# ForJadeForest/DistillCLIP

Hardware: AMD Instinct MI355X
Metric: image-text pairs/sec (distill step) (higher is better)
Workload: dtype bf16; 1 GPU; l_clip.yaml dual distill: ViT-B/32 CLIP teacher -> weight-shared ViT(6x768,24h,R2) + text(4x768,12h,R2) students, 224px/77tok, losses out_l1+out_cos+0.1*cos_diff, fwd+loss+bwd+AdamW; global_batch=512, batch_per_gpu=512, parallelism=dp1, gradient_exchange=none, negatives=local (reference training_step semantics), optimizer_in_step=True, teacher_residual=fp16, saved_gelu_derivative=u8 fixed point, clock_probe=True

## Files before the change

distillclip_amd/csrc/gemm_common.h:

```cpp
#pragma once
#include <math.h>
#include <stdlib.h>
#include "common.h"
#include <type_traits>

namespace dgemm {

constexpr int BM = 128, BN = 128, BK = 64;
constexpr int SUB = 1024;
constexpr int HT = 16384;

inline unsigned long long* g_gemm_stamps = nullptr;

struct GemmNT {
    const bf16_t* A; int64_t lda;
    const bf16_t* B; int64_t ldb;
    void* C; int64_t ldc;
    int M, N, K;
    float alpha;
    const float* bias;
    const void* aux_in;
    void* aux_out;
    const void* residual; int64_t ldr;
    int row_group; const float* rowadd;
// ... 76 lines not shown
        float dg[8];
#pragma unroll
        for (int e = 0; e < 8; ++e) {
            const float sg = __builtin_amdgcn_rcpf(1.f + __expf(-1.702f * v[e]));
            dg[e] = fmaf(1.702f * v[e] * sg, 1.f - sg, sg);
            v[e] *= sg;
        }
        if (LEAN || p.aux_out) *(uint2*)((uint8_t*)p.aux_out + o) = uint2{dg_pack4(dg[0], dg[1], dg[2], dg[3]), dg_pack4(dg[4], dg[5], dg[6], dg[7])};
    }
    if (MODE == 3 || (!LEAN && p.residual)) {
        if (OUT == 2) {
            const f16x8 r = sd.rh;
#pragma unroll
            for (int e = 0; e < 8; ++e) v[e] += (float)r[e];
        } else {
            float4 r0, r1;
            if (OUT == 1) { r0 = sd.r0; r1 = sd.r1; }
            else {
                const float* rp = (const float*)p.residual + orr;
                r0 = *(const float4*)rp; r1 = *(const float4*)(rp + 4);
            }
            v[0] += r0.x; v[1] += r0.y; v[2] += r0.z; v[3] += r0.w; v[4] += r1.x; v[5] += r1.y; v[6] += r1.z; v[7] += r1.w;
        }
    }
    if (OUT == 1) {
        float* cp = (float*)p.C + o;
        *(float4*)cp = float4{v[0], v[1], v[2], v[3]};
        *(float4*)(cp + 4) = float4{v[4], v[5], v[6], v[7]};
    } else if (OUT == 2) {
        f16x8 ov;
#pragma unroll
        for (int e = 0; e < 8; ++e) ov[e] = (_Float16)v[e];
        *(f16x8*)((_Float16*)p.C + o) = ov;
    } else {
        bf16x8 ov;
#pragma unroll
        for (int e = 0; e < 8; ++e) ov[e] = f2bf(v[e]);
        *(bf16x8*)((bf16_t*)p.C + o) = ov;
    }
    if (CSUM_ALWAYS || (OUT == 0 && (MODE == 2 || (MODE == 0 && p.colsum)))) {
#pragma unroll
        for (int e = 0; e < 8; ++e) csum[e] += v[e];
    }
}

#define WAIT_VMCNT(n) asm volatile("s_waitcnt vmcnt(" #n ")" ::: "memory")
#define WAIT_LGKM0() asm volatile("s_waitcnt lgkmcnt(0)" ::: "memory")

__device__ __forceinline__ void wg_stamp(unsigned long long* const& stamps, const int& tid, int k) {
    if (stamps && tid == 0) {
        if (k == 3) WAIT_VMCNT(0);
        stamps[6 * (int64_t)blockIdx.x + k] = __builtin_readcyclecounter();
        if (k == 0) stamps[6 * (int64_t)blockIdx.x + 4] = __builtin_amdgcn_s_memrealtime();
        if (k == 3) stamps[6 * (int64_t)blockIdx.x + 5] = __builtin_amdgcn_s_memrealtime();
    }
}

__device__ __forceinline__ void mfma_4x4(f32x4 (&acc)[4][4], const bf16x8 (&a)[4], const bf16x8 (&b)[4]) {
#pragma unroll
    for (int i = 0; i < 4; ++i)
#pragma unroll
        for (int j = 0; j < 4; ++j) acc[i][j] = __builtin_amdgcn_mfma_f32_16x16x32_bf16(a[i], b[j], acc[i][j], 0, 0, 0);
}

template <bool SWAP>
__device__ __forceinline__ f32x4 mfma_rc(bf16x8 rowf, bf16x8 colf, f32x4 c) {
    return SWAP ? __builtin_amdgcn_mfma_f32_16x16x32_bf16(colf, rowf, c, 0, 0, 0) : __builtin_amdgcn_mfma_f32_16x16x32_bf16(rowf, colf, c, 0, 0, 0);
}
#define PHASE_MFMA(SWAP, acc, R0, RT, af, b0, b1)                                                                         \
    do {                                                                                                                  \
        __builtin_amdgcn_s_barrier();                                                                                     \
        __builtin_amdgcn_s_setprio(1);                                                                                    \
        _Pragma("unroll") for (int kb_ = 0; kb_ < 2; ++kb_)                                                               \
            _Pragma("unroll") for (int i_ = 0; i_ < (RT); ++i_) {                                                         \
                _Pragma("unroll") for (int j_ = 0; j_ < 2; ++j_)                                                          \
                    acc[(R0) + i_][j_] = mfma_rc<SWAP>(af[i_][kb_], b0[j_][kb_], acc[(R0) + i_][j_]);                     \
                _Pragma("unroll") for (int j_ = 0; j_ < 2; ++j_)                                                          \
                    acc[(R0) + i_][2 + j_] = mfma_rc<SWAP>(af[i_][kb_], b1[j_][kb_], acc[(R0) + i_][2 + j_]);             \
            }                                                                                                             \
        __builtin_amdgcn_s_setprio(0);                                                                                    \
        __builtin_amdgcn_s_barrier();                                                                                     \
    } while (0)

template <int NI, int LD>
__device__ __forceinline__ void stage_acc(float* cs, const f32x4 (*acc)[4], int row0, int col0, int lane) {
#pragma unroll
    for (int i = 0; i < NI; ++i)
#pragma unroll
        for (int j = 0; j < 4; ++j)
#pragma unroll
            for (int r = 0; r < 4; ++r) cs[(row0 + i * 16 + (lane >> 4) * 4 + r) * LD + col0 + j * 16 + (lane & 15)] = acc[i][j][r];
}

}
```

distillclip_amd/csrc/gemm_nt.hip:

```cpp

#include "gemm_common.h"
#include <atomic>

using namespace dgemm;

namespace {

constexpr int TILE_BYTES = (BM / 16) * (BK / 32) * SUB;
constexpr int CLD = BN + 4;
constexpr int NT_LDS = (4 * TILE_BYTES > BM * CLD * 4) ? 4 * TILE_BYTES : BM * CLD * 4;


__device__ __forceinline__ void stage_operand(const bf16_t* __restrict__ G, int64_t ld, int row0, int rows_max,
                                              int k0, char* lds_tile, int wave, int lane) {
    const int L = lane * 16;
    const int X = swz(L);
    const int r = X >> 6, c = (X >> 4) & 3;
#pragma unroll
    for (int s = 0; s < 4; ++s) {
        const int sub = wave * 4 + s;
        const int rb = sub >> 1, kb = sub & 1;
        int row = row0 + rb * 16 + r;
        row = row < rows_max ? row : rows_max - 1;
        const bf16_t* src = G + (int64_t)row * ld + (k0 + kb * 32 + c * 8);
        __builtin_amdgcn_global_load_lds((gbl_void*)src, (lds_void*)(lds_tile + sub * SUB), 16, 0, 0);
    }
}

template <int ACT, int OUT>
__global__ __launch_bounds__(256) void gemm_nt_kernel(GemmNT p) {
    extern __shared__ __attribute__((aligned(16))) char smem[];
    const int tid = threadIdx.x, lane = tid & 63;
    const int wave = __builtin_amdgcn_readfirstlane(tid >> 6);
    const int wm = wave >> 1, wn = wave & 1;

    const int nwg = p.tiles_m * p.tiles_n;
    const int t = xcd_remap(blockIdx.x, nwg);
    const int tm = t / p.tiles_n, tn = t % p.tiles_n;
    const int m0 = tm * BM, n0 = tn * BN;

    char* As = smem;
    char* Bs = smem + 2 * TILE_BYTES;

    f32x4 acc[4][4];
#pragma unroll
    for (int i = 0; i < 4; ++i)
#pragma unroll
        for (int j = 0; j < 4; ++j) acc[i][j] = f32x4{0.f, 0.f, 0.f, 0.f};

    const int nk = p.K / BK;
    stage_operand(p.A, p.lda, m0, p.M, 0, As, wave, lane);
    stage_operand(p.B, p.ldb, n0, p.N, 0, Bs, wave, lane);

    const int fragoff = swz((lane & 15) * 64 + (lane >> 4) * 16);

    for (int kt = 0; kt < nk; ++kt) {
        __syncthreads();
        if (kt + 1 < nk) {
            const int nb = (kt + 1) & 1;
            stage_operand(p.A, p.lda, m0, p.M, (kt + 1) * BK, As + nb * TILE_BYTES, wave, lane);
            stage_operand(p.B, p.ldb, n0, p.N, (kt + 1) * BK, Bs + nb * TILE_BYTES, wave, lane);
        }
        const char* a_t = As + (kt & 1) * TILE_BYTES;
        const char* b_t = Bs + (kt & 1) * TILE_BYTES;
#pragma unroll
        for (int kb = 0; kb < 2; ++kb) {
            bf16x8 af[4], bfr[4];
#pragma unroll
            for (int i = 0; i < 4; ++i)
                af[i] = *(const bf16x8*)(a_t + ((wm * 4 + i) * 2 + kb) * SUB + fragoff);
#pragma unroll
            for (int j = 0; j < 4; ++j)
                bfr[j] = *(const bf16x8*)(b_t + ((wn * 4 + j) * 2 + kb) * SUB + fragoff);
            mfma_4x4(acc, af, bfr);
        }
    }

    __syncthreads();
    float* cs = (float*)smem;
    stage_acc<4, CLD>(cs, acc, wm * 64, wn * 64, lane);
    __syncthreads();
    const int cc = (tid & 15) * 8;
    const int col = n0 + cc;
    const bool col_ok = col < p.N;
    float bias[8], csum[8];
#pragma unroll
    for (int e = 0; e < 8; ++e) { bias[e] = 0.f; csum[e] = 0.f; }
    if (p.bias && col_ok) {
        const float4 b0 = *(const float4*)(p.bias + col), b1 = *(const float4*)(p.bias + col + 4);
        bias[0] = b0.x; bias[1] = b0.y; bias[2] = b0.z; bias[3] = b0.w; bias[4] = b1.x; bias[5] = b1.y; bias[6] = b1.z; bias[7] = b1.w;
    }
#pragma unroll
    for (int it = 0; it < 8; ++it) {
        const int rl = (tid >> 4) + it * 16;
        const int row = m0 + rl;
        if (row >= p.M || !col_ok) break;
        const float4 c0 = *(const float4*)(cs + rl * CLD + cc), c1 = *(const float4*)(cs + rl * CLD + cc + 4);
        float v[8] = {c0.x, c0.y, c0.z, c0.w, c1.x, c1.y, c1.z, c1.w};
        const int64_t o = (int64_t)row * p.ldc + col, orr = (int64_t)row * p.ldr + col;
        EpiSide sd;
        epilogue_load_side<ACT, OUT>(p, o, orr, sd);
        epilogue_vec8<ACT, OUT, 0, true>(p, v, row, col, o, orr, bias, csum, sd);
    }
    if (p.colsum) {
        __syncthreads();
#pragma unroll
        for (int e = 0; e < 8; ++e) cs[(tid >> 4) * CLD + cc + e] = csum[e];
        __syncthreads();
        if (tid < BN && n0 + tid < p.N) {
            float x = 0.f;
#pragma unroll
            for (int r = 0; r < 16; ++r) x += cs[r * CLD + tid];
            unsafeAtomicAdd(p.colsum + n0 + tid, x);
        }
    }
}


constexpr int nt256_lds(int mi) { return 2 * (2 * HT + 2 * (mi * 16 * BK * 2)); }

__device__ __forceinline__ void stage_half_perm(const bf16_t* __restrict__ G, int64_t ld, int row0, int rows_max, int k0,
                                                char* buf, int wave, int lane) {
    const int L = lane * 16;
    const int X = swz(L);
    const int r = X >> 6, c = (X >> 4) & 3;
    const int j = wave & 3;
    int row = row0 + (wave >> 2) * 64 + (j >> 1) * 32 + (r >> 2) * 8 + (j & 1) * 4 + (r & 3);
    row = row < rows_max ? row : rows_max - 1;
    const bf16_t* src = G + (int64_t)row * ld + k0 + c * 8;
    __builtin_amdgcn_global_load_lds((gbl_void*)src, (lds_void*)(buf + (wave * 2 + 0) * SUB), 16, 0, 0);
    __builtin_amdgcn_global_load_lds((gbl_void*)(src + 32), (lds_void*)(buf + (wave * 2 + 1) * SUB), 16, 0, 0);
}

template <int RH>
__device__ __forceinline__ void stage_rowhalf(const bf16_t* __restrict__ G, int64_t ld, int m0, int rows_max, int k0,
                                              char* abase, int hta, int dn, int wave, int lane) {
    const int L = lane * 16;
    const int X = swz(L);
    const int r = X >> 6, c = (X >> 4) & 3;
    constexpr int AROWS = RH * 32;
    {
        const int wv = RH == 3 ? wave % 6 : wave;
        const int g = wv / RH, i = wv % RH + dn * RH;
        int row = m0 + g * AROWS + i * 16 + r;
        row = row < rows_max ? row : rows_max - 1;
        const bf16_t* src = G + (int64_t)row * ld + k0 + c * 8;
        char* dst = abase + g * hta + (i * 2) * SUB;
        __builtin_amdgcn_global_load_lds((gbl_void*)src, (lds_void*)dst, 16, 0, 0);
        __builtin_amdgcn_global_load_lds((gbl_void*)(src + 32), (lds_void*)(dst + SUB), 16, 0, 0);
    }
    if (RH == 5) {
        const int e = wave & 3, rbk = 8 + (e >> 1), kb = e & 1;
        const int g = rbk / RH, i = rbk % RH + dn * RH;
        int row = m0 + g * AROWS + i * 16 + r;
        row = row < rows_max ? row : rows_max - 1;
        const bf16_t* src = G + (int64_t)row * ld + k0 + kb * 32 + c * 8;
        __builtin_amdgcn_global_load_lds((gbl_void*)src, (lds_void*)(abase + g * hta + (i * 2 + kb) * SUB), 16, 0, 0);
    }
}

__device__ __forceinline__ float row16_sum(float x) {
    auto dpp = [](float v, auto ctrl) {
        return __builtin_bit_cast(float, __builtin_amdgcn_update_dpp(0, __builtin_bit_cast(int, v), decltype(ctrl)::value, 0xf, 0xf, false));
    };
    x += dpp(x, std::integral_constant<int, 0xB1>{});
    x += dpp(x, std::integral_constant<int, 0x4E>{});
    x += dpp(x, std::integral_constant<int, 0x141>{});
    x += dpp(x, std::integral_constant<int, 0x140>{});
    return x;
}

template <int ACT, int OUT, int MI>
__global__ __launch_bounds__(512) void gemm_nt256_kernel(GemmNT p) {
    extern __shared__ __attribute__((aligned(16))) char smem[];
    constexpr int RH = MI / 2;
    constexpr int AROWS = MI * 16;
    constexpr int HTA = AROWS * BK * 2;
    constexpr int PAR = nt256_lds(MI) / 2;
    constexpr int BMT = 2 * AROWS;
    const int tid = threadIdx.x, lane = tid & 63;
    const int wave = __builtin_amdgcn_readfirstlane(tid >> 6);
    const int wr = wave >> 2, wc = wave & 3;

    const int nwg = p.tiles_m * p.tiles_n;
    const int nk = p.K / BK;
    const int nload = 4 * nk;
    int m0, n0;
    auto locate = [&](int tl) {
        const int t = xcd_remap(tl, nwg);
        int tm, tn;
        if (p.group_n >= p.tiles_n) { tm = t / p.tiles_n; tn = t % p.tiles_n; }
        else {
            const int per = p.tiles_m * p.group_n;
            const int gi = t / per, rem = t - gi * per;
            const int left = p.tiles_n - gi * p.group_n;
            const int gw = left < p.group_n ? left : p.group_n;
            tm = rem / gw; tn = gi * p.group_n + rem % gw;
        }
// ... 61 lines not shown
    if (wr == 0) __builtin_amdgcn_s_barrier();
    wg_stamp(p.stamps, tid, 2);
    const int g = lane >> 4, rl = lane & 15;

    const int colb = n0 + wc * 64 + g * 8;
    float bias[2][8], csum[2][8];
#pragma unroll
    for (int jp = 0; jp < 2; ++jp) {
#pragma unroll
        for (int e = 0; e < 8; ++e) { bias[jp][e] = 0.f; csum[jp][e] = 0.f; }
        const int col = colb + jp * 32;
        if (p.bias && col < p.N) {
            const float4 q0 = *(const float4*)(p.bias + col), q1 = *(const float4*)(p.bias + col + 4);
            bias[jp][0] = q0.x; bias[jp][1] = q0.y; bias[jp][2] = q0.z; bias[jp][3] = q0.w;
            bias[jp][4] = q1.x; bias[jp][5] = q1.y; bias[jp][6] = q1.z; bias[jp][7] = q1.w;
        }
    }
    constexpr bool OUT_F32 = OUT == 1;
    constexpr bool SIDE = OUT != 0 || ACT == 3 || ACT == 4;
    constexpr int NU = 2 * MI;
    constexpr int BU = !SIDE ? NU : (OUT_F32 ? ((ACT == 3 || ACT == 4) ? 4 : (MI == 8 ? 8 : (MI == 6 ? 6 : 5))) : (MI == 10 ? 10 : NU));
    static_assert(NU % BU == 0, "batch size must divide the unit count");
    EpiSide side[SIDE ? BU : 1];
    const int row0 = m0 + wr * AROWS + rl;
    const int64_t o0 = (int64_t)row0 * p.ldc + colb, r0off = (int64_t)row0 * p.ldr + colb;
    const int64_t ostep = 16 * p.ldc, rstep = 16 * p.ldr;
    const bool full = m0 + BMT <= p.M && n0 + 256 <= p.N;
    auto run_units = [&](auto mode_tag) {
        constexpr int MODE = decltype(mode_tag)::value;
#pragma unroll
        for (int ub = 0; ub < NU; ub += BU) {
            if (SIDE) {
#pragma unroll
                for (int u = ub; u < ub + BU; ++u) {
                    const int i = u >> 1, jp = u & 1;
                    if (full || (row0 + i * 16 < p.M && colb + jp * 32 < p.N))
                        epilogue_load_side<ACT, OUT>(p, o0 + i * ostep + jp * 32, r0off + i * rstep + jp * 32, side[u - ub]);
                }
            }
#pragma unroll
            for (int u = ub; u < ub + BU; ++u) {
                const int i = u >> 1, jp = u & 1;
                const int row = row0 + i * 16, col = colb + jp * 32;
                if (full || (row < p.M && col < p.N)) {
                    float v[8];
#pragma unroll
                    for (int r = 0; r < 4; ++r) { v[r] = acc[i][2 * jp][r]; v[4 + r] = acc[i][2 * jp + 1][r]; }
                    epilogue_vec8<ACT, OUT, MODE>(p, v, row, col, o0 + i * ostep + jp * 32, r0off + i * rstep + jp * 32, bias[jp], csum[jp],
                                                      side[SIDE ? u - ub : 0]);
                }
            }
        }
    };
    const bool lean = p.row_group == 0 && ((ACT == 5 || ACT == 6) ? p.aux_out != nullptr : p.aux_out == nullptr) && (OUT != 0 ? p.residual != nullptr : p.residual == nullptr);
    if constexpr (OUT != 0) {
        if (lean) run_units(std::integral_constant<int, 3>{});
        else run_units(std::integral_constant<int, 0>{});
    } else if constexpr (ACT == 3 || ACT == 4) {
        if (lean && p.colsum) run_units(std::integral_constant<int, 2>{});
        else run_units(std::integral_constant<int, 0>{});
    } else {
        if (lean && !p.colsum) run_units(std::integral_constant<int, 1>{});
        else if (lean) run_units(std::integral_constant<int, 2>{});
        else run_units(std::integral_constant<int, 0>{});
    }
    if (OUT == 0 && p.colsum) {
        float* cs = (float*)smem;
#pragma unroll
        for (int jp = 0; jp < 2; ++jp)
#pragma unroll
            for (int e = 0; e < 8; ++e) {
                const float x = row16_sum(csum[jp][e]);
                if (rl == 0) cs[wr * 256 + wc * 64 + jp * 32 + g * 8 + e] = x;
            }
        WAIT_LGKM0();
        __builtin_amdgcn_s_barrier();
        const int tc = wave * 64 + lane;
        if (tc < 256 && n0 + tc < p.N) unsafeAtomicAdd(p.colsum + n0 + tc, cs[tc] + cs[256 + tc]);
    }
    wg_stamp(p.stamps, tid, 3);
    if (p.clk && blockIdx.x == 0 && tid == 0) { p.clk[2] = __builtin_amdgcn_s_memtime(); p.clk[3] = __builtin_amdgcn_s_memrealtime(); }
}

bool use_256(const GemmNT& p) {
    static const int mode = [] { const char* e = getenv("DCLIP_GEMM256"); return e ? atoi(e) : 1; }();
    return mode != 0 && p.M >= 1024 && p.N >= 256;
}

std::atomic<unsigned long long*> g_clock_buf{nullptr};
std::atomic<long long> g_clock_cap{0};
std::atomic<long long> g_clock_count{0};
inline unsigned long long* next_clock_slot() {
    unsigned long long* buf = g_clock_buf.load(std::memory_order_acquire);
    const long long cap = g_clock_cap.load(std::memory_order_relaxed);
    if (!buf || cap <= 0) return nullptr;
    return buf + 4 * (g_clock_count.fetch_add(1, std::memory_order_relaxed) % cap);
}

int tile_height_mi(const GemmNT& p, int act, int out) {
    static const int mode320 = [] { const char* e = getenv("DCLIP_GEMM320"); return e ? atoi(e) : 1; }();
    if (!mode320) return 8;
    if (mode320 == 2) return 10;
    if (mode320 == 6) return 6;
    const int tn = (p.N + 255) / 256;
    const double nkt = (double)(p.K / BK), e8 = out == 1 ? 40000.0 : out == 2 ? 24000.0 : (act == 0 || act == 4 ? 9500.0 : 14000.0);
    auto cost = [&](int rows, double per_kt, double escale) {
        const int tmx = (p.M + rows - 1) / rows;
        return (double)((tmx * tn + 255) / 256) * (3300.0 + nkt * per_kt + escale * e8);
    };
    const double c8 = cost(256, 2750.0, 1.0), c10 = cost(320, 3200.0, 1.25), c6 = cost(192, 2150.0, 0.75);
    int mi = 8;
    if (c10 < c8) mi = 10;
    if (c6 < (mi == 10 ? c10 : c8) * 0.97) mi = 6;
    return mi;
}

int raster_group_n(const GemmNT& p) {
    const int tn = p.tiles_n, ntiles = p.tiles_m * p.tiles_n;
    const double panel = 512.0 * (double)p.K, a_bytes = 2.0 * (double)p.M * (double)p.K;
    double best = 0.0; int best_g = tn;
    for (int g = 1; g <= tn; ++g) {
        const int ngroups = (tn + g - 1) / g;
        const double b_term = (g * panel <= 2.5e6) ? 8.0 * g * panel * (ngroups > 8 ? ngroups / 8.0 : 1.0)
                                                   : (double)ntiles / 32.0 * g * panel;
        const double cost = a_bytes * ngroups + b_term;
        if (g == 1 || cost < best * 0.999) { best = cost; best_g = g; }
    }
    return best_g;
}

template <int ACT, int MI>
void launch_nt256(const GemmNT& p, int out, hipStream_t st) {
    const dim3 grid(p.tiles_m * p.tiles_n), block(512);
    constexpr size_t lds = nt256_lds(MI) + 16;
    if (out == 1) { if constexpr (ACT == 0) hipLaunchKernelGGL((gemm_nt256_kernel<0, 1, MI>), grid, block, lds, st, p); }
    else if (out == 2) { if constexpr (ACT == 0) hipLaunchKernelGGL((gemm_nt256_kernel<0, 2, MI>), grid, block, lds, st, p); }
    else hipLaunchKernelGGL((gemm_nt256_kernel<ACT, 0, MI>), grid, block, lds, st, p);
}

template <int ACT>
int launch_nt(GemmNT p, int out, hipStream_t st) {
    if constexpr (ACT != 0) { if (out == 2) { dclip_set_error("dclip_gemm_nt: f16 output needs act = DCLIP_ACT_NONE"); return DCLIP_EINVAL; } }
    if (use_256(p) && !(out != 0 && p.colsum) && (ACT == 0 || out == 0)) {
        const int mi = tile_height_mi(p, ACT, out);
        p.tiles_m = (p.M + mi * 32 - 1) / (mi * 32); p.tiles_n = (p.N + 255) / 256;
        p.clk = next_clock_slot();
        p.group_n = raster_group_n(p);
        if (mi == 10) launch_nt256<ACT, 10>(p, out, st);
        else if (mi == 6) launch_nt256<ACT, 6>(p, out, st);
        else launch_nt256<ACT, 8>(p, out, st);
        return dclip_check_launch("dclip_gemm_nt");
    }
    const int grid = p.tiles_m * p.tiles_n;
    const size_t lds = NT_LDS;
    if (out == 1) hipLaunchKernelGGL((gemm_nt_kernel<ACT, 1>), dim3(grid), dim3(256), lds, st, p);
    else if (out == 2) { if constexpr (ACT == 0) hipLaunchKernelGGL((gemm_nt_kernel<0, 2>), dim3(grid), dim3(256), lds, st, p); }
    else hipLaunchKernelGGL((gemm_nt_kernel<ACT, 0>), dim3(grid), dim3(256), lds, st, p);
    return dclip_check_launch("dclip_gemm_nt");
}

}

extern "C" int dclip_trace_gemm_stamps(void* buf) { g_gemm_stamps = (unsigned long long*)buf; return 0; }
extern "C" int64_t dclip_trace_gemm_clock(void* buf, int64_t cap) {
    const long long n = g_clock_count.exchange(0, std::memory_order_relaxed);
    g_clock_cap.store(buf ? (long long)cap : 0, std::memory_order_relaxed);
    g_clock_buf.store((unsigned long long*)buf, std::memory_order_release);
    return (int64_t)n;
}

extern "C" int dclip_gemm_nt(const void* A, int64_t lda, const void* B, int64_t ldb, void* C, int64_t ldc,
                             int64_t M, int64_t N, int64_t K, float alpha, const float* bias, int act,
                             const void* aux_in, void* aux_out, const void* residual, int64_t ldr, int out_dtype,
                             int64_t row_group, const float* rowadd, float* colsum_acc, void* stream) {
    DCLIP_REQUIRE(A && B && C, "dclip_gemm_nt: null operand");
    DCLIP_REQUIRE(M > 0 && N > 0 && K > 0, "dclip_gemm_nt: empty problem M=%ld N=%ld K=%ld", (long)M, (long)N, (long)K);
    DCLIP_REQUIRE(K % BK == 0, "dclip_gemm_nt: K=%ld must be a multiple of %d", (long)K, BK);
    DCLIP_REQUIRE(lda % 8 == 0 && ldb % 8 == 0 && ((uintptr_t)A % 16) == 0 && ((uintptr_t)B % 16) == 0,
                  "dclip_gemm_nt: operand rows must be 16-byte aligned (lda=%ld ldb=%ld)", (long)lda, (long)ldb);
    DCLIP_REQUIRE(N % 8 == 0 && ldc % 8 == 0 && ((uintptr_t)C % 16) == 0, "dclip_gemm_nt: N and ldc must be multiples of 8 and C 16-byte aligned (N=%ld ldc=%ld)", (long)N, (long)ldc);
    DCLIP_REQUIRE(out_dtype >= 0 && out_dtype <= 2, "dclip_gemm_nt: bad output dtype %d (0 bf16, 1 f32, 2 f16)", out_dtype);
    DCLIP_REQUIRE(!residual || (ldr % (out_dtype == 2 ? 8 : 4) == 0 && ((uintptr_t)residual % 16) == 0), "dclip_gemm_nt: residual rows must be 16-byte aligned");
    DCLIP_REQUIRE(act >= 0 && act <= 6, "dclip_gemm_nt: bad activation code %d", act);
    DCLIP_REQUIRE(out_dtype != 2 || act == 0, "dclip_gemm_nt: f16 output needs act = DCLIP_ACT_NONE");
    DCLIP_REQUIRE((act != DCLIP_ACT_DGELU && act != DCLIP_ACT_MULAUX) || aux_in, "dclip_gemm_nt: DGELU / MULAUX need aux_in");
    DCLIP_REQUIRE(!aux_in || ((uintptr_t)aux_in % 16) == 0, "dclip_gemm_nt: aux_in must be 16-byte aligned");
    DCLIP_REQUIRE(!aux_out || ((uintptr_t)aux_out % 16) == 0, "dclip_gemm_nt: aux_out must be 16-byte aligned");
    DCLIP_REQUIRE(row_group == 0 || rowadd, "dclip_gemm_nt: row_group needs rowadd");
    DCLIP_REQUIRE(M < (1LL << 31) && N < (1LL << 31), "dclip_gemm_nt: dimension overflow");
    GemmNT p;
    p.A = (const bf16_t*)A; p.lda = lda; p.B = (const bf16_t*)B; p.ldb = ldb; p.C = C; p.ldc = ldc;
    p.M = (int)M; p.N = (int)N; p.K = (int)K; p.alpha = alpha; p.bias = bias;
    p.aux_in = aux_in; p.aux_out = aux_out; p.residual = residual; p.ldr = ldr;
    p.row_group = (int)row_group; p.rowadd = rowadd; p.colsum = colsum_acc;
    p.tiles_m = (int)((M + BM - 1) / BM); p.tiles_n = (int)((N + BN - 1) / BN);
    p.stamps = g_gemm_stamps;
    p.group_n = 1 << 30;
    p.clk = nullptr;
    hipStream_t st = (hipStream_t)stream;
    const int out_f32 = out_dtype == 1;
    const double aux_b = (act == DCLIP_ACT_MULAUX || act == DCLIP_ACT_GELU_SAVE || act == DCLIP_ACT_QUICKGELU_SAVE) ? 1.0 : 2.0;
    TraceScope tr(DCLIP_TRACE_GEMM_NT, 2.0 * (double)M * (double)N * (double)K,
                  2.0 * ((double)M * K + (double)N * K) + ((out_f32 ? 4.0 : 2.0) + (residual ? (out_dtype == 2 ? 2.0 : 4.0) : 0.0) + (aux_in ? aux_b : 0.0) + (aux_out ? aux_b : 0.0)) * (double)M * N,
                  stream, (int)M, (int)N, (int)K,
                  act + 8 * (out_f32 != 0) + 16 * (residual != nullptr) + 32 * (colsum_acc != nullptr) + 64 * (out_dtype == 2));
    switch (act) {
        case 0: return launch_nt<0>(p, out_dtype, st);
        case 1: return launch_nt<1>(p, out_dtype, st);
        case 2: return launch_nt<2>(p, out_dtype, st);
        case 3: return launch_nt<3>(p, out_dtype, st);
        case 4: return launch_nt<4>(p, out_dtype, st);
        case 5: return launch_nt<5>(p, out_dtype, st);
        default: return launch_nt<6>(p, out_dtype, st);
    }
}
```

include/dclip.h:

```cpp
#ifndef DCLIP_H
#define DCLIP_H
#include <stddef.h>
#include <stdint.h>
#ifdef __cplusplus
extern "C" {
#endif

#define DCLIP_OK 0
#define DCLIP_EINVAL (-1)
#define DCLIP_ELAUNCH (-2)

int dclip_version(void);
int dclip_runtime_check(void);
const char* dclip_arch(void);
const char* dclip_last_error_string(void);

#define DCLIP_ACT_NONE 0
#define DCLIP_ACT_QUICKGELU 1
#define DCLIP_ACT_GELU 2
#define DCLIP_ACT_DGELU 3
#define DCLIP_ACT_MULAUX 4
#define DCLIP_ACT_GELU_SAVE 5
#define DCLIP_ACT_QUICKGELU_SAVE 6
#define DCLIP_OUT_BF16 0
#define DCLIP_OUT_F32 1
#define DCLIP_OUT_F16 2

int dclip_gemm_nt(const void* A, int64_t lda, const void* B, int64_t ldb, void* C, int64_t ldc,
                  int64_t M, int64_t N, int64_t K, float alpha, const float* bias, int act,
                  const void* aux_in, void* aux_out, const void* residual, int64_t ldr, int out_dtype,
                  int64_t row_group, const float* rowadd, float* colsum_acc, void* stream);

size_t dclip_gemm_tn_workspace_bytes(void);
int64_t dclip_gemm_tn_atomic_fallbacks(void);
int dclip_gemm_tn_acc(const void* A, int64_t lda, const void* B, int64_t ldb, float* dW, int64_t ldo,
                      int64_t M, int64_t P, int64_t Q, int splits, void* workspace, size_t ws_bytes, void* stream);

int dclip_colsum_acc(const void* X, int64_t ld, float* db, int64_t M, int64_t N, void* stream);

int dclip_layernorm_fwd(const float* x, int64_t ldx, const int32_t* row_index, const float* gamma, const float* beta,
                        void* y, int64_t ldy, int out_f32, float* mean, float* rstd, int64_t M, int64_t D, float eps,
                        void* stream);
int dclip_layernorm_fwd_f16(const void* x, int64_t ldx, const int32_t* row_index, const float* gamma, const float* beta,
                            void* y, int64_t ldy, int out_dtype, float* mean, float* rstd, int64_t M, int64_t D, float eps,
                            void* stream);
int dclip_layernorm_bwd(const void* dy, int64_t lddy, int dy_f32, const float* x, int64_t ldx, const int32_t* row_index,
                        const float* gamma, const float* mean, const float* rstd, float* dx_acc, int64_t lddx,
                        void* dx_bf16, int64_t lddb, float* dgamma, float* dbeta, float* colsum_acc, int64_t M, int64_t D,
                        void* stream);

int dclip_attn_nt(const void* A, int64_t lda, const void* Bm, int64_t ldb, void* C, int out_f32, int64_t B, int64_t H,
                  int64_t N, int64_t Np, int64_t hd, float alpha, void* stream);
int dclip_attn_nn(const void* A, const void* Bm, int64_t ldb, void* C, int64_t ldc, int64_t B, int64_t H, int64_t N,
                  int64_t Np, int64_t hd, float alpha, int a_blocked, void* stream);
int dclip_attn_tn(const void* A, const void* Bm, int64_t ldb, void* C, int64_t ldc, int64_t B, int64_t H, int64_t N,
                  int64_t Np, int64_t hd, float alpha, int a_blocked, void* stream);
int dclip_attn_fused_fwd(const void* qkv, int64_t ldq, void* ctx, int64_t ldc, int64_t B, int64_t H, int64_t N, int64_t hd,
                         float scale, int causal, void* stream);
int dclip_attn_stream_fwd(const void* qkv, int64_t ldq, void* ctx, int64_t ldc, int64_t B, int64_t H, int64_t N, int64_t hd,
                          float scale, void* stream);
int dclip_attn_softmax_fwd(const float* S, const float* Wl, const float* Ww, void* P, void* R, int64_t B, int64_t H,
                           int64_t N, int64_t Np, int causal, void* stream);
int dclip_attn_softmax_bwd(const void* dR, const void* P, const void* S, int scores_bf16, const float* Wl, const float* Ww,
                           void* dS, float* dWl, float* dWw, int64_t B, int64_t H, int64_t N, int64_t Np, void* stream);
int dclip_attn_mix_supported(int64_t H, int64_t N, int64_t hd);
size_t dclip_attn_mix_bwd_workspace_bytes(int64_t B, int64_t H, int64_t N);
void dclip_attn_mix_debug_stamps(void* fwd, void* bwd_a, void* bwd_b);
int dclip_attn_mix_fwd(const void* qkv, int64_t ld, const float* Wl, const float* Ww, void* R, float* stats, int64_t B, int64_t H,
                       int64_t N, int64_t Np, int64_t hd, float scale, void* stream);
int dclip_attn_mix_bwd(const void* qkv, int64_t ld, const void* dO, int64_t ldo, const float* Wl, const float* Ww,
                       const float* stats, void* dS, float* dWl, float* dWw, void* workspace, size_t ws_bytes, int64_t B, int64_t H,
                       int64_t N, int64_t Np, int64_t hd, float scale, void* stream);
int dclip_attn_nn_rows(const void* A, const void* Bm, int64_t ldb, void* C, int64_t ldc, int64_t B, int64_t H, int64_t N, int64_t Np,
                       int64_t hd, float alpha, int a_blocked, const int32_t* pick, int fill_zero, void* stream);
int dclip_attn_tn_rows(const void* A, const void* Bm, int64_t ldb, void* C, int64_t ldc, int64_t B, int64_t H, int64_t N, int64_t Np,
                       int64_t hd, float alpha, int a_blocked, const int32_t* pick, void* stream);
int dclip_attn_fused_fwd_rows(const void* qkv, int64_t ldq, void* ctx, int64_t ldc, int64_t B, int64_t H, int64_t N, int64_t hd,
                              float scale, int causal, const int32_t* pick, void* stream);
int dclip_attn_mix_fwd_rows(const void* qkv, int64_t ld, const float* Wl, const float* Ww, void* R, float* stats, int64_t B, int64_t H,
                            int64_t N, int64_t Np, int64_t hd, float scale, const int32_t* pick, void* stream);
int dclip_attn_mix_bwd_rows(const void* qkv, int64_t ld, const void* dO, int64_t ldo, const float* Wl, const float* Ww,
                            const float* stats, void* dS, float* dWl, float* dWw, void* workspace, size_t ws_bytes, int64_t B, int64_t H,
                            int64_t N, int64_t Np, int64_t hd, float scale, const int32_t* pick, void* stream);
int dclip_attn_maps_fwd(const void* qkv, int64_t ld, const float* Wl, float* score_map, float* prob_map, int64_t B, int64_t H, int64_t N,
                        int64_t hd, float scale, int causal, void* stream);
size_t dclip_attn_maps_bwd_workspace_bytes(int64_t B, int64_t H, int64_t N);
int dclip_attn_maps_bwd(const void* qkv, int64_t ld, const float* Wl, const float* d_score_map, const float* d_prob_map, void* dS,
                        int ds_blocked, float* dWl, void* workspace, size_t ws_bytes, int64_t B, int64_t H, int64_t N, int64_t Np,
                        int64_t hd, float scale, int causal, void* stream);

int dclip_cast_bf16(const float* src, void* dst, int64_t n, void* stream);
int dclip_cast_f16_f32(const void* src, float* dst, int64_t n, void* stream);
int dclip_axpy_f32(float* dst, const float* src, void* dst_bf16, int64_t n, float* colsum_acc, int64_t D, void* stream);
int dclip_cast_transpose_bf16_multi(const float* const* W, void* const* Wb, void* const* Wt, const int64_t* R, const int64_t* C,
                                    int64_t n, void* stream);
int dclip_im2row(const float* img, void* rows, int64_t B, int64_t C, int64_t res, int64_t patch, int cls_rows, void* stream);
int dclip_im2row_ld(const float* img, void* rows, int64_t ldk, int64_t B, int64_t C, int64_t res, int64_t patch, int cls_rows,
                    void* stream);
int dclip_token_table(const float* pos, const float* cls, const float* bias, float* out, int64_t ntok, int64_t D, void* stream);
int dclip_token_table_bwd(const float* tok_sum, float* dpos, float* dcls, float* dbias, int64_t ntok, int64_t D, int has_cls,
                          void* stream);
int dclip_batch_sum_acc(const float* G, float* out, int64_t B, int64_t N, int64_t D, void* stream);
int dclip_embed_gather(const int64_t* ids, int64_t id_stride, const float* table, const float* pos, void* out, int out_dtype,
                       int64_t rows, int64_t N, int64_t D, void* stream);
int dclip_embed_scatter_add(const int64_t* ids, const void* dx, int dx_f32, float* dtable, int64_t rows, int64_t D,
                            int64_t vocab, void* stream);
int dclip_pick_index(const int64_t* ids, int64_t id_stride, int32_t* idx, int64_t B, int64_t N, void* stream);
int dclip_adamw(float* p, float* g, float* m, float* v, int64_t n, float lr, float beta1, float beta2, float eps,
                float weight_decay, int64_t step, int zero_grad, void* stream);
#define DCLIP_ADAMW_MAX_RANGES 24
int dclip_adamw_multi(float* const* p, float* const* g, float* const* m, float* const* v, const int64_t* n, int32_t count, float lr,
                      float beta1, float beta2, float eps, float weight_decay, int64_t step, int zero_grad, void* stream);
int dclip_adamw_multi_scaled(float* const* p, float* const* g, float* const* m, float* const* v, const int64_t* n, int32_t count,
                             float lr, float beta1, float beta2, float eps, float weight_decay, int64_t step, int zero_grad,
// ... 122 lines not shown
```

Before: 18660 pairs/s.

## Add 64x64 row-tile NT GEMM kernel with cost-model routing

Adds a new small-tile (64x64) NT GEMM kernel that uses a deep global-to-LDS ring buffer and the shared epilogue. A cost model that estimates waves of workgroups, per-k-tile cost and epilogue cost now picks between this kernel and the existing 128-square or 256-wide kernels. The aim is better CU occupancy and less tail waste on GEMMs that produce too few large tiles to fill the GPU. The risk is that the heuristic constants mis-route shapes to the smaller tile, which reuses data less. A route query API is also exported.

```diff
diff --git a/distillclip_amd/csrc/gemm_common.h b/distillclip_amd/csrc/gemm_common.h
--- a/distillclip_amd/csrc/gemm_common.h
+++ b/distillclip_amd/csrc/gemm_common.h
@@ -182,12 +182,12 @@
         __builtin_amdgcn_s_barrier();                                                                                     \
     } while (0)
 
-template <int NI, int LD>
-__device__ __forceinline__ void stage_acc(float* cs, const f32x4 (*acc)[4], int row0, int col0, int lane) {
+template <int NI, int LD, int NJ = 4>
+__device__ __forceinline__ void stage_acc(float* cs, const f32x4 (*acc)[NJ], int row0, int col0, int lane) {
 #pragma unroll
     for (int i = 0; i < NI; ++i)
 #pragma unroll
-        for (int j = 0; j < 4; ++j)
+        for (int j = 0; j < NJ; ++j)
 #pragma unroll
             for (int r = 0; r < 4; ++r) cs[(row0 + i * 16 + (lane >> 4) * 4 + r) * LD + col0 + j * 16 + (lane & 15)] = acc[i][j][r];
 }
diff --git a/distillclip_amd/csrc/gemm_nt.hip b/distillclip_amd/csrc/gemm_nt.hip
--- a/distillclip_amd/csrc/gemm_nt.hip
+++ b/distillclip_amd/csrc/gemm_nt.hip
@@ -1,5 +1,6 @@
 
 #include "gemm_common.h"
+#include "gemm_nt_rows.h"
 #include <atomic>
 
 using namespace dgemm;
@@ -341,10 +342,11 @@
     if (p.clk && blockIdx.x == 0 && tid == 0) { p.clk[2] = __builtin_amdgcn_s_memtime(); p.clk[3] = __builtin_amdgcn_s_memrealtime(); }
 }
 
-bool use_256(const GemmNT& p) {
+int gemm256_mode() {
     static const int mode = [] { const char* e = getenv("DCLIP_GEMM256"); return e ? atoi(e) : 1; }();
-    return mode != 0 && p.M >= 1024 && p.N >= 256;
-}
+    return mode;
+}
+bool use_256(const GemmNT& p) { return gemm256_mode() != 0 && p.M >= 1024 && p.N >= 256; }
 
 std::atomic<unsigned long long*> g_clock_buf{nullptr};
 std::atomic<long long> g_clock_cap{0};
@@ -356,22 +358,50 @@
     return buf + 4 * (g_clock_count.fetch_add(1, std::memory_order_relaxed) % cap);
 }
 
+double epilogue_256sq(int act, int out) { return out == 1 ? 40000.0 : out == 2 ? 24000.0 : (act == 0 || act == 4 ? 9500.0 : 14000.0); }
+double nt256_cost(const GemmNT& p, int act, int out, int mi) {
+    const int rows = 32 * mi, tn = (p.N + 255) / 256, tmx = (p.M + rows - 1) / rows;
+    const double per_kt = mi == 10 ? 3200.0 : mi == 6 ? 2150.0 : 2750.0, escale = mi == 10 ? 1.25 : mi == 6 ? 0.75 : 1.0;
+    return (double)((tmx * tn + 255) / 256) * (3300.0 + (double)(p.K / BK) * per_kt + escale * epilogue_256sq(act, out));
+}
+int gemm320_mode() {
+    static const int mode320 = [] { const char* e = getenv("DCLIP_GEMM320"); return e ? atoi(e) : 1; }();
+    return mode320;
+}
 int tile_height_mi(const GemmNT& p, int act, int out) {
-    static const int mode320 = [] { const char* e = getenv("DCLIP_GEMM320"); return e ? atoi(e) : 1; }();
+    const int mode320 = gemm320_mode();
     if (!mode320) return 8;
     if (mode320 == 2) return 10;
     if (mode320 == 6) return 6;
-    const int tn = (p.N + 255) / 256;
-    const double nkt = (double)(p.K / BK), e8 = out == 1 ? 40000.0 : out == 2 ? 24000.0 : (act == 0 || act == 4 ? 9500.0 : 14000.0);
-    auto cost = [&](int rows, double per_kt, double escale) {
-        const int tmx = (p.M + rows - 1) / rows;
-        return (double)((tmx * tn + 255) / 256) * (3300.0 + nkt * per_kt + escale * e8);
-    };
-    const double c8 = cost(256, 2750.0, 1.0), c10 = cost(320, 3200.0, 1.25), c6 = cost(192, 2150.0, 0.75);
+    auto cost = [&](int mi) { return nt256_cost(p, act, out, mi); };
+    const double c8 = cost(8), c10 = cost(10), c6 = cost(6);
     int mi = 8;
     if (c10 < c8) mi = 10;
     if (c6 < (mi == 10 ? c10 : c8) * 0.97) mi = 6;
     return mi;
+}
+
+constexpr double ROUND_TRIP = 2000.0, ROWS_KT_ALONE = 650.0, ROWS_KT_SHARED = 540.0, SQ128_KT_ALONE = 1400.0, SQ128_KT_BUSY = 1100.0, EPI_FIXED = 1500.0;
+int gemm_rows_mode() {
+    static const int mode = [] { const char* e = getenv("DCLIP_GEMM_ROWS"); return e ? atoi(e) : 1; }();
+    return mode;
+}
+double small_cost(const GemmNT& p, int act, int out, int bm, int bn, int wg_per_cu, double kt_alone, double kt_shared) {
+    const long long nwg = (long long)((p.M + bm - 1) / bm) * ((p.N + bn - 1) / bn);
+    const long long rounds = (nwg + 256 * wg_per_cu - 1) / (256 * wg_per_cu);
+    const long long share = nwg > 256 ? wg_per_cu : 1;
+    const double per_kt = kt_alone > share * kt_shared ? kt_alone : share * kt_shared;
+    return (double)rounds * (ROUND_TRIP + (double)(p.K / BK) * per_kt + EPI_FIXED + epilogue_256sq(act, out) * (double)(bm * bn) / 65536.0);
+}
+int route_nt(const GemmNT& p, int act, int out) {
+    const bool large = use_256(p) && !(out != 0 && p.colsum) && (act == 0 || out == 0);
+    const int mi = large ? tile_height_mi(p, act, out) : 0;
+    const int mode = gemm_rows_mode();
+    if (mode == 0 || gemm256_mode() == 0 || (large && gemm320_mode() != 1)) return mi;
+    if (mode == 2) return 1;
+    const double c_rows = small_cost(p, act, out, ROWS_BM, ROWS_BN, rows_wg_per_cu(), ROWS_KT_ALONE, ROWS_KT_SHARED);
+    const double c_other = large ? nt256_cost(p, act, out, mi) : small_cost(p, act, out, BM, BN, 2, SQ128_KT_ALONE, SQ128_KT_BUSY);
+    return c_rows < c_other ? 1 : mi;
 }
 
 int raster_group_n(const GemmNT& p) {
@@ -400,8 +430,9 @@
 template <int ACT>
 int launch_nt(GemmNT p, int out, hipStream_t st) {
     if constexpr (ACT != 0) { if (out == 2) { dclip_set_error("dclip_gemm_nt: f16 output needs act = DCLIP_ACT_NONE"); return DCLIP_EINVAL; } }
-    if (use_256(p) && !(out != 0 && p.colsum) && (ACT == 0 || out == 0)) {
-        const int mi = tile_height_mi(p, ACT, out);
+    const int mi = route_nt(p, ACT, out);
+    if (mi == 1) return launch_nt_rows(p, ACT, out, st);
+    if (mi != 0) {
         p.tiles_m = (p.M + mi * 32 - 1) / (mi * 32); p.tiles_n = (p.N + 255) / 256;
         p.clk = next_clock_slot();
         p.group_n = raster_group_n(p);
@@ -418,6 +449,18 @@
     return dclip_check_launch("dclip_gemm_nt");
 }
 
+}
+
+extern "C" int dclip_gemm_nt_route(int64_t M, int64_t N, int64_t K, int act, int out_dtype, int has_colsum, int32_t* route) {
+    DCLIP_REQUIRE(route, "dclip_gemm_nt_route: null result");
+    DCLIP_REQUIRE(M > 0 && N > 0 && K > 0 && K % BK == 0 && M < (1LL << 31) && N < (1LL << 31), "dclip_gemm_nt_route: bad problem M=%ld N=%ld K=%ld", (long)M, (long)N, (long)K);
+    DCLIP_REQUIRE(act >= 0 && act <= 6 && out_dtype >= 0 && out_dtype <= 2, "dclip_gemm_nt_route: bad activation / output code");
+    GemmNT p{};
+    p.M = (int)M; p.N = (int)N; p.K = (int)K;
+    static float some_colsum;
+    p.colsum = has_colsum ? &some_colsum : nullptr;
+    *route = route_nt(p, act, out_dtype);
+    return DCLIP_OK;
 }
 
 extern "C" int dclip_trace_gemm_stamps(void* buf) { g_gemm_stamps = (unsigned long long*)buf; return 0; }
diff --git a/distillclip_amd/csrc/gemm_nt_rows.h b/distillclip_amd/csrc/gemm_nt_rows.h
--- /dev/null
+++ b/distillclip_amd/csrc/gemm_nt_rows.h
@@ -0,0 +1,11 @@
+#pragma once
+#include "gemm_common.h"
+
+namespace dgemm {
+
+constexpr int ROWS_BM = 64, ROWS_BN = 64;
+
+int launch_nt_rows(GemmNT p, int act, int out, hipStream_t st);
+int rows_wg_per_cu();
+
+}
diff --git a/distillclip_amd/csrc/gemm_nt_rows.hip b/distillclip_amd/csrc/gemm_nt_rows.hip
--- /dev/null
+++ b/distillclip_amd/csrc/gemm_nt_rows.hip
@@ -0,0 +1,179 @@
+#include "gemm_common.h"
+#include "gemm_nt_rows.h"
+
+using namespace dgemm;
+
+namespace {
+
+#ifndef DCLIP_ROWS_DEPTH
+#define DCLIP_ROWS_DEPTH 4
+#endif
+constexpr int ROWS_DEPTH = DCLIP_ROWS_DEPTH;
+constexpr int RSTAGE = 2 * (ROWS_BM / 16) * (BK / 32) * SUB;
+constexpr int RCLD = ROWS_BN + 4;
+constexpr int ROWS_LDS = ROWS_DEPTH * RSTAGE;
+static_assert(ROWS_DEPTH >= 3 && ROWS_DEPTH <= 10, "ring depth");
+static_assert(ROWS_LDS >= ROWS_BM * RCLD * 4, "the C tile is staged in the ring");
+
+template <int N>
+__device__ __forceinline__ void wait_vm() { asm volatile("s_waitcnt vmcnt(%0)" ::"n"(N) : "memory"); }
+
+template <int Y>
+__device__ __forceinline__ void wait_stages_younger(int y) {
+    if (y >= Y) wait_vm<4 * Y>();
+    else if constexpr (Y > 0) wait_stages_younger<Y - 1>(y);
+}
+
+template <int ACT, int OUT>
+__global__ __launch_bounds__(256) void gemm_nt_rows_kernel(GemmNT p) {
+    extern __shared__ __attribute__((aligned(16))) char smem[];
+    const int tid = threadIdx.x, lane = tid & 63;
+    const int wave = __builtin_amdgcn_readfirstlane(tid >> 6);
+    const int wm = wave >> 1, wn = wave & 1;
+
+    const int nwg = p.tiles_m * p.tiles_n;
+    const int t = xcd_remap(blockIdx.x, nwg);
+    const int tm = t / p.tiles_n, tn = t % p.tiles_n;
+    const int m0 = tm * ROWS_BM, n0 = tn * ROWS_BN;
+
+    const bf16_t *srcA, *srcB;
+    {
+        const int X = swz(lane * 16);
+        const int r = X >> 6, c = (X >> 4) & 3;
+        int ra = m0 + wave * 16 + r, rb = n0 + wave * 16 + r;
+        ra = ra < p.M ? ra : p.M - 1;
+        rb = rb < p.N ? rb : p.N - 1;
+        srcA = p.A + (int64_t)ra * p.lda + c * 8;
+        srcB = p.B + (int64_t)rb * p.ldb + c * 8;
+    }
+    auto issue = [&](int kt, int slot) {
+        char* st = smem + slot * RSTAGE + wave * 2 * SUB;
+        const bf16_t *a = srcA + kt * BK, *b = srcB + kt * BK;
+        __builtin_amdgcn_global_load_lds((gbl_void*)a, (lds_void*)st, 16, 0, 0);
+        __builtin_amdgcn_global_load_lds((gbl_void*)(a + 32), (lds_void*)(st + SUB), 16, 0, 0);
+        __builtin_amdgcn_global_load_lds((gbl_void*)b, (lds_void*)(st + 8 * SUB), 16, 0, 0);
+        __builtin_amdgcn_global_load_lds((gbl_void*)(b + 32), (lds_void*)(st + 9 * SUB), 16, 0, 0);
+    };
+
+    const int nk = p.K / BK;
+    const int npro = nk < ROWS_DEPTH - 1 ? nk : ROWS_DEPTH - 1;
+    for (int s = 0; s < npro; ++s) issue(s, s);
+
+    f32x4 acc[2][2];
+#pragma unroll
+    for (int i = 0; i < 2; ++i)
+#pragma unroll
+        for (int j = 0; j < 2; ++j) acc[i][j] = f32x4{0.f, 0.f, 0.f, 0.f};
+
+    const int fragoff = swz((lane & 15) * 64 + (lane >> 4) * 16);
+    const int a_off = wm * 4 * SUB + fragoff, b_off = (8 + wn * 4) * SUB + fragoff;
+
+    int slot = 0, fill = ROWS_DEPTH - 1;
+    for (int kt = 0; kt < nk; ++kt) {
+        wait_stages_younger<ROWS_DEPTH - 2>(nk - 1 - kt);
+        __builtin_amdgcn_s_barrier();
+        if (kt + ROWS_DEPTH - 1 < nk) issue(kt + ROWS_DEPTH - 1, fill);
+        const char* st = smem + slot * RSTAGE;
+        bf16x8 af[2][2], bfr[2][2];
+#pragma unroll
+        for (int kb = 0; kb < 2; ++kb)
+#pragma unroll
+            for (int i = 0; i < 2; ++i) {
+                af[kb][i] = *(const bf16x8*)(st + a_off + (i * 2 + kb) * SUB);
+                bfr[kb][i] = *(const bf16x8*)(st + b_off + (i * 2 + kb) * SUB);
+            }
+        WAIT_LGKM0();
+#pragma unroll
+        for (int kb = 0; kb < 2; ++kb)
+#pragma unroll
+            for (int i = 0; i < 2; ++i)
+#pragma unroll
+                for (int j = 0; j < 2; ++j) acc[i][j] = mfma_rc<false>(af[kb][i], bfr[kb][j], acc[i][j]);
+        slot = slot + 1 == ROWS_DEPTH ? 0 : slot + 1;
+        fill = fill + 1 == ROWS_DEPTH ? 0 : fill + 1;
+    }
+
+    __syncthreads();
+    float* cs = (float*)smem;
+    stage_acc<2, RCLD, 2>(cs, acc, wm * 32, wn * 32, lane);
+    __syncthreads();
+
+    const int cc = (tid & 7) * 8;
+    const int col = n0 + cc;
+    const bool col_ok = col < p.N;
+    float bias[8], csum[8];
+#pragma unroll
+    for (int e = 0; e < 8; ++e) { bias[e] = 0.f; csum[e] = 0.f; }
+    if (p.bias && col_ok) {
+        const float4 b0 = *(const float4*)(p.bias + col), b1 = *(const float4*)(p.bias + col + 4);
+        bias[0] = b0.x; bias[1] = b0.y; bias[2] = b0.z; bias[3] = b0.w; bias[4] = b1.x; bias[5] = b1.y; bias[6] = b1.z; bias[7] = b1.w;
+    }
+    const int rl0 = tid >> 3;
+    EpiSide sd[2];
+#pragma unroll
+    for (int it = 0; it < 2; ++it) {
+        const int row = m0 + rl0 + it * 32;
+        if (row < p.M && col_ok) epilogue_load_side<ACT, OUT>(p, (int64_t)row * p.ldc + col, (int64_t)row * p.ldr + col, sd[it]);
+    }
+#pragma unroll
+    for (int it = 0; it < 2; ++it) {
+        const int rl = rl0 + it * 32;
+        const int row = m0 + rl;
+        if (row < p.M && col_ok) {
+            float* cp = cs + rl * RCLD + cc;
+            const float4 c0 = *(const float4*)cp, c1 = *(const float4*)(cp + 4);
+            float v[8] = {c0.x, c0.y, c0.z, c0.w, c1.x, c1.y, c1.z, c1.w};
+            epilogue_vec8<ACT, OUT, 0, false>(p, v, row, col, (int64_t)row * p.ldc + col, (int64_t)row * p.ldr + col, bias, csum, sd[it]);
+            if (p.colsum) {
+                *(float4*)cp = float4{v[0], v[1], v[2], v[3]};
+                *(float4*)(cp + 4) = float4{v[4], v[5], v[6], v[7]};
+            }
+        }
+    }
+    if (p.colsum) {
+        __syncthreads();
+        if (tid < ROWS_BN && n0 + tid < p.N) {
+            const int rows = p.M - m0 < ROWS_BM ? p.M - m0 : ROWS_BM;
+            float x = 0.f;
+#pragma unroll
+            for (int g = 0; g < 16; ++g) {
+                float s = 0.f;
+#pragma unroll
+                for (int it = 0; it < 4; ++it)
+                    if (g + it * 16 < rows) s += cs[(g + it * 16) * RCLD + tid];
+                x += s;
+            }
+            unsafeAtomicAdd(p.colsum + n0 + tid, x);
+        }
+    }
+}
+
+}
+
+namespace dgemm {
+
+template <int ACT>
+static void launch_rows_act(const GemmNT& p, int out, hipStream_t st) {
+    const dim3 grid(p.tiles_m * p.tiles_n), block(256);
+    if (out == 1) hipLaunchKernelGGL((gemm_nt_rows_kernel<ACT, 1>), grid, block, ROWS_LDS, st, p);
+    else if (out == 2) { if constexpr (ACT == 0) hipLaunchKernelGGL((gemm_nt_rows_kernel<0, 2>), grid, block, ROWS_LDS, st, p); }
+    else hipLaunchKernelGGL((gemm_nt_rows_kernel<ACT, 0>), grid, block, ROWS_LDS, st, p);
+}
+
+int rows_wg_per_cu() { return (160 * 1024) / ROWS_LDS >= 2 ? 2 : 1; }
+
+int launch_nt_rows(GemmNT p, int act, int out, hipStream_t st) {
+    p.tiles_m = (p.M + ROWS_BM - 1) / ROWS_BM; p.tiles_n = (p.N + ROWS_BN - 1) / ROWS_BN;
+    switch (act) {
+        case 0: launch_rows_act<0>(p, out, st); break;
+        case 1: launch_rows_act<1>(p, out, st); break;
+        case 2: launch_rows_act<2>(p, out, st); break;
+        case 3: launch_rows_act<3>(p, out, st); break;
+        case 4: launch_rows_act<4>(p, out, st); break;
+        case 5: launch_rows_act<5>(p, out, st); break;
+        default: launch_rows_act<6>(p, out, st); break;
+    }
+    return dclip_check_launch("dclip_gemm_nt");
+}
+
+}
diff --git a/include/dclip.h b/include/dclip.h
--- a/include/dclip.h
+++ b/include/dclip.h
@@ -30,6 +30,7 @@
                   int64_t M, int64_t N, int64_t K, float alpha, const float* bias, int act,
                   const void* aux_in, void* aux_out, const void* residual, int64_t ldr, int out_dtype,
                   int64_t row_group, const float* rowadd, float* colsum_acc, void* stream);
+int dclip_gemm_nt_route(int64_t M, int64_t N, int64_t K, int act, int out_dtype, int has_colsum, int32_t* route);
 
 size_t dclip_gemm_tn_workspace_bytes(void);
 int64_t dclip_gemm_tn_atomic_fallbacks(void);
```

After: 18780 pairs/s, median of 6. Within noise of the previous version (+0.6%).

## Add multi-stage LDS ring pipeline and 64-row tiles to fallback NT GEMM

Applied to the files above, without the earlier changes.

Replaces the double-buffered 128x128 fallback NT GEMM with a templated kernel that uses a 3-stage LDS ring. It relies on counted vmcnt waits instead of __syncthreads, and spreads the global-to-LDS loads for the next stage between MFMA groups. When the problem has few tiles it picks 64-row tiles to put more workgroups on the GPU. This targets load latency and under-occupancy on small GEMMs that do not take the 256-wide path, at the cost of more LDS per workgroup and hand-tuned wait counts that must stay exactly right.

```diff
diff --git a/distillclip_amd/csrc/gemm_nt.hip b/distillclip_amd/csrc/gemm_nt.hip
--- a/distillclip_amd/csrc/gemm_nt.hip
+++ b/distillclip_amd/csrc/gemm_nt.hip
@@ -8,27 +8,39 @@
 
 constexpr int TILE_BYTES = (BM / 16) * (BK / 32) * SUB;
 constexpr int CLD = BN + 4;
-constexpr int NT_LDS = (4 * TILE_BYTES > BM * CLD * 4) ? 4 * TILE_BYTES : BM * CLD * 4;
-
-
-__device__ __forceinline__ void stage_operand(const bf16_t* __restrict__ G, int64_t ld, int row0, int rows_max,
-                                              int k0, char* lds_tile, int wave, int lane) {
-    const int L = lane * 16;
-    const int X = swz(L);
+
+
+template <int NP>
+__device__ __forceinline__ void nt_sources(const bf16_t* __restrict__ G, int64_t ld, int row0, int rows_max, int wave, int lane,
+                                           const char* (&src)[NP]) {
+    const int X = swz(lane * 16);
     const int r = X >> 6, c = (X >> 4) & 3;
 #pragma unroll
-    for (int s = 0; s < 4; ++s) {
-        const int sub = wave * 4 + s;
+    for (int s = 0; s < NP; ++s) {
+        const int sub = wave * NP + s;
         const int rb = sub >> 1, kb = sub & 1;
         int row = row0 + rb * 16 + r;
         row = row < rows_max ? row : rows_max - 1;
-        const bf16_t* src = G + (int64_t)row * ld + (k0 + kb * 32 + c * 8);
-        __builtin_amdgcn_global_load_lds((gbl_void*)src, (lds_void*)(lds_tile + sub * SUB), 16, 0, 0);
-    }
-}
-
-template <int ACT, int OUT>
+        src[s] = (const char*)(G + (int64_t)row * ld + (kb * 32 + c * 8));
+    }
+}
+
+constexpr int RING = 3;
+constexpr int nt_stage_bytes(int mi) { return mi * 4 * SUB + TILE_BYTES; }
+constexpr int nt_lds(int stages, int mi) { return stages * nt_stage_bytes(mi) > 32 * mi * CLD * 4 ? stages * nt_stage_bytes(mi) : 32 * mi * CLD * 4; }
+
+template <int N>
+__device__ __forceinline__ void wait_vmcnt() { asm volatile("s_waitcnt vmcnt(%0)" ::"n"(N) : "memory"); }
+
+template <int ACT, int OUT, int STAGES, int MI>
 __global__ __launch_bounds__(256) void gemm_nt_kernel(GemmNT p) {
+    static_assert(STAGES >= 2 && STAGES <= 4, "the counted waits below cover 2 to 4 stages");
+    static_assert(MI == 4 || MI == 2, "128- or 64-row tiles");
+    constexpr int BMT = 32 * MI;
+    constexpr int NP = MI + 4;
+    constexpr int STAGE = nt_stage_bytes(MI);
+    constexpr int A_BYTES = MI * 4 * SUB;
+    constexpr bool SPREAD = STAGES > 2;
     extern __shared__ __attribute__((aligned(16))) char smem[];
     const int tid = threadIdx.x, lane = tid & 63;
     const int wave = __builtin_amdgcn_readfirstlane(tid >> 6);
@@ -37,48 +49,86 @@
     const int nwg = p.tiles_m * p.tiles_n;
     const int t = xcd_remap(blockIdx.x, nwg);
     const int tm = t / p.tiles_n, tn = t % p.tiles_n;
-    const int m0 = tm * BM, n0 = tn * BN;
-
-    char* As = smem;
-    char* Bs = smem + 2 * TILE_BYTES;
-
-    f32x4 acc[4][4];
-#pragma unroll
-    for (int i = 0; i < 4; ++i)
+    const int m0 = tm * BMT, n0 = tn * BN;
+
+    f32x4 acc[MI][4];
+#pragma unroll
+    for (int i = 0; i < MI; ++i)
 #pragma unroll
         for (int j = 0; j < 4; ++j) acc[i][j] = f32x4{0.f, 0.f, 0.f, 0.f};
 
     const int nk = p.K / BK;
-    stage_operand(p.A, p.lda, m0, p.M, 0, As, wave, lane);
-    stage_operand(p.B, p.ldb, n0, p.N, 0, Bs, wave, lane);
+    const char* src_a[MI];
+    const char* src_b[4];
+    nt_sources<MI>(p.A, p.lda, m0, p.M, wave, lane, src_a);
+    nt_sources<4>(p.B, p.ldb, n0, p.N, wave, lane, src_b);
+    auto piece = [&](int q, int kt, int s) {
+        const char* src = (q < MI ? src_a[q < MI ? q : 0] : src_b[q < MI ? 0 : q - MI]) + (int64_t)kt * (BK * 2);
+        char* dst = smem + s * STAGE + (q < MI ? (wave * MI + q) * SUB : A_BYTES + (wave * 4 + q - MI) * SUB);
+        __builtin_amdgcn_global_load_lds((gbl_void*)src, (lds_void*)dst, 16, 0, 0);
+    };
+    wg_stamp(p.stamps, tid, 0);
+#pragma unroll
+    for (int s = 0; s < STAGES - 1; ++s)
+        if (s < nk) {
+#pragma unroll
+            for (int q = 0; q < NP; ++q) piece(q, s, s);
+        }
 
     const int fragoff = swz((lane & 15) * 64 + (lane >> 4) * 16);
 
-    for (int kt = 0; kt < nk; ++kt) {
-        __syncthreads();
-        if (kt + 1 < nk) {
-            const int nb = (kt + 1) & 1;
-            stage_operand(p.A, p.lda, m0, p.M, (kt + 1) * BK, As + nb * TILE_BYTES, wave, lane);
-            stage_operand(p.B, p.ldb, n0, p.N, (kt + 1) * BK, Bs + nb * TILE_BYTES, wave, lane);
-        }
-        const char* a_t = As + (kt & 1) * TILE_BYTES;
-        const char* b_t = Bs + (kt & 1) * TILE_BYTES;
+    int rd = 0, wr = STAGES - 1;
+    auto k_tile = [&](int kt, auto req_tag) {
+        constexpr bool REQ = decltype(req_tag)::value;
+        const int after = nk - 1 - kt;
+        if (REQ || after >= STAGES - 2) wait_vmcnt<NP * (STAGES - 2)>();
+        else if (STAGES == 4 && after == 1) wait_vmcnt<NP>();
+        else wait_vmcnt<0>();
+        WAIT_LGKM0();
+        __builtin_amdgcn_s_barrier();
+        if (kt == 0) wg_stamp(p.stamps, tid, 1);
+        if (REQ && !SPREAD) {
+#pragma unroll
+            for (int q = 0; q < NP; ++q) piece(q, kt + STAGES - 1, wr);
+        }
+        const char* a_t = smem + rd * STAGE;
+        const char* b_t = a_t + A_BYTES;
+        bf16x8 af[2][MI], bfr[2][4];
 #pragma unroll
         for (int kb = 0; kb < 2; ++kb) {
-            bf16x8 af[4], bfr[4];
-#pragma unroll
-            for (int i = 0; i < 4; ++i)
-                af[i] = *(const bf16x8*)(a_t + ((wm * 4 + i) * 2 + kb) * SUB + fragoff);
+#pragma unroll
+            for (int i = 0; i < MI; ++i)
+                af[kb][i] = *(const bf16x8*)(a_t + ((wm * MI + i) * 2 + kb) * SUB + fragoff);
 #pragma unroll
             for (int j = 0; j < 4; ++j)
-                bfr[j] = *(const bf16x8*)(b_t + ((wn * 4 + j) * 2 + kb) * SUB + fragoff);
-            mfma_4x4(acc, af, bfr);
-        }
-    }
+                bfr[kb][j] = *(const bf16x8*)(b_t + ((wn * 4 + j) * 2 + kb) * SUB + fragoff);
+        }
+#pragma unroll
+        for (int g = 0; g < 8; ++g) {
+            const int kb = g >> 2;
+#pragma unroll
+            for (int u = 0; u < MI; ++u) {
+                const int x = (g & 3) * MI + u, i = x >> 2, j = x & 3;
+                acc[i][j] = __builtin_amdgcn_mfma_f32_16x16x32_bf16(af[kb][i], bfr[kb][j], acc[i][j], 0, 0, 0);
+            }
+            if (REQ && SPREAD && g < NP) piece(g, kt + STAGES - 1, wr);
+            if (SPREAD) __builtin_amdgcn_sched_barrier(0);
+        }
+        __builtin_amdgcn_sched_barrier(0);
+        asm volatile("s_nop 7");
+        mfma_keep_alive(af[0]); mfma_keep_alive(af[1]); mfma_keep_alive(bfr[0]); mfma_keep_alive(bfr[1]);
+        wr = rd;
+        rd = rd + 1 == STAGES ? 0 : rd + 1;
+    };
+    const int nreq = nk - (STAGES - 1);
+    int kt = 0;
+    for (; kt < nreq; ++kt) k_tile(kt, std::true_type{});
+    for (; kt < nk; ++kt) k_tile(kt, std::false_type{});
+    wg_stamp(p.stamps, tid, 2);
 
     __syncthreads();
     float* cs = (float*)smem;
-    stage_acc<4, CLD>(cs, acc, wm * 64, wn * 64, lane);
+    stage_acc<MI, CLD>(cs, acc, wm * (BMT / 2), wn * 64, lane);
     __syncthreads();
     const int cc = (tid & 15) * 8;
     const int col = n0 + cc;
@@ -91,7 +141,7 @@
         bias[0] = b0.x; bias[1] = b0.y; bias[2] = b0.z; bias[3] = b0.w; bias[4] = b1.x; bias[5] = b1.y; bias[6] = b1.z; bias[7] = b1.w;
     }
 #pragma unroll
-    for (int it = 0; it < 8; ++it) {
+    for (int it = 0; it < BMT / 16; ++it) {
         const int rl = (tid >> 4) + it * 16;
         const int row = m0 + rl;
         if (row >= p.M || !col_ok) break;
@@ -114,6 +164,7 @@
             unsafeAtomicAdd(p.colsum + n0 + tid, x);
         }
     }
+    wg_stamp(p.stamps, tid, 3);
 }
 
 
@@ -346,6 +397,13 @@
     return mode != 0 && p.M >= 1024 && p.N >= 256;
 }
 
+constexpr int NT64_TILES = 128;
+int nt_instance(const GemmNT& p) {
+    static const int mode = [] { const char* e = getenv("DCLIP_GEMM_RING"); return e ? atoi(e) : 1; }();
+    const int tiles = p.tiles_m * p.tiles_n;
+    return mode == 0 || tiles > 256 ? 0 : (tiles <= NT64_TILES ? 2 : 1);
+}
+
 std::atomic<unsigned long long*> g_clock_buf{nullptr};
 std::atomic<long long> g_clock_cap{0};
 std::atomic<long long> g_clock_count{0};
@@ -395,6 +453,16 @@
     if (out == 1) { if constexpr (ACT == 0) hipLaunchKernelGGL((gemm_nt256_kernel<0, 1, MI>), grid, block, lds, st, p); }
     else if (out == 2) { if constexpr (ACT == 0) hipLaunchKernelGGL((gemm_nt256_kernel<0, 2, MI>), grid, block, lds, st, p); }
     else hipLaunchKernelGGL((gemm_nt256_kernel<ACT, 0, MI>), grid, block, lds, st, p);
+}
+
+template <int ACT, int STAGES, int MI>
+void launch_nt128(GemmNT p, int out, hipStream_t st) {
+    p.tiles_m = (p.M + 32 * MI - 1) / (32 * MI);
+    const dim3 grid(p.tiles_m * p.tiles_n), block(256);
+    constexpr size_t lds = nt_lds(STAGES, MI);
+    if (out == 1) hipLaunchKernelGGL((gemm_nt_kernel<ACT, 1, STAGES, MI>), grid, block, lds, st, p);
+    else if (out == 2) { if constexpr (ACT == 0) hipLaunchKernelGGL((gemm_nt_kernel<0, 2, STAGES, MI>), grid, block, lds, st, p); }
+    else hipLaunchKernelGGL((gemm_nt_kernel<ACT, 0, STAGES, MI>), grid, block, lds, st, p);
 }
 
 template <int ACT>
@@ -410,11 +478,10 @@
         else launch_nt256<ACT, 8>(p, out, st);
         return dclip_check_launch("dclip_gemm_nt");
     }
-    const int grid = p.tiles_m * p.tiles_n;
-    const size_t lds = NT_LDS;
-    if (out == 1) hipLaunchKernelGGL((gemm_nt_kernel<ACT, 1>), dim3(grid), dim3(256), lds, st, p);
-    else if (out == 2) { if constexpr (ACT == 0) hipLaunchKernelGGL((gemm_nt_kernel<0, 2>), dim3(grid), dim3(256), lds, st, p); }
-    else hipLaunchKernelGGL((gemm_nt_kernel<ACT, 0>), dim3(grid), dim3(256), lds, st, p);
+    const int inst = nt_instance(p);
+    if (inst == 2) launch_nt128<ACT, RING, 2>(p, out, st);
+    else if (inst == 1) launch_nt128<ACT, RING, 4>(p, out, st);
+    else launch_nt128<ACT, 2, 4>(p, out, st);
     return dclip_check_launch("dclip_gemm_nt");
 }
 
```

New measurement: 18910 pairs/s before, 18940 pairs/s after, median of 4. Within noise of the previous version (+0.2%).
